# jhuldr/BrainFM

Measured on AMD Instinct MI355X. Metric: voxels/sec whole-volume multi-task inference, 256^3 tiled, higher is better.
Workload: dtype f16x3-split (fp32-grade); 1 GPU; 256^3 volume, reference tiling win160/stride80 -> 27 tiles, UNet3D f64 x6 levels, 9 heads (69 ch), fused tail + deformed atlas + on-device stitch of 17 keys; stitched_keys=17, mfma_passes=3, submission=hipGraph replay per tile shape, parallelism=tiles sharded over 1 rank(s), gather to rank 0, tiles_in_flight_per_gpu=2

## Files before the change

### brainfm_amd/csrc/conv3d_wino.hip

```cpp
#include "wino_shared.h"
#include <cstdlib>
#include <type_traits>

namespace {

typedef _Float16 half8 __attribute__((ext_vector_type(8)));
typedef _Float16 half4 __attribute__((ext_vector_type(4)));
typedef float floatx16 __attribute__((ext_vector_type(16)));

constexpr int KC = 16;
constexpr int NTHR = 256;
constexpr int MLD = 33;

struct WinoParams {
    const float* A;
    int CA, D, H, W;
    const float *scale, *shift, *bound;
    int G;
    const uint4* wp;
    int wexp, Cout;
    float slope;
    float* out;
    int accum;
    int TD, TH, TW, HT, PW;
// ... 530 lines not shown
        *reinterpret_cast<float4*>(p.pool_out + dbase + off1) = v1;
    }
    if (tid < 64) {
        const size_t d = (size_t)mt * p.Cout + nt * 64 + tid, s = (size_t)rp * p.Cout + nt * 64 + tid;
        if (p.rsum != nullptr) { p.rsum[d] = p.rsum[s]; p.rsq[d] = p.rsq[s]; p.rmn[d] = p.rmn[s]; p.rmx[d] = p.rmx[s]; }
        if (p.prsum != nullptr) { p.prsum[d] = p.prsum[s]; p.prsq[d] = p.prsq[s]; p.prmn[d] = p.prmn[s]; p.prmx[d] = p.prmx[s]; }
    }
}

template <class Pred>
__device__ __forceinline__ int wino_compact(int nMt, Pred pred, int* __restrict__ list, int* sh) {
    const int tid = threadIdx.x, lane = tid & 63, wv = tid >> 6;
    if (tid == 0) sh[16] = 0;
    __syncthreads();
    for (int b0 = 0; b0 < nMt; b0 += 1024) {
        const int mt = b0 + tid;
        const bool keep = mt < nMt && pred(mt);
        const unsigned long long bal = __ballot(keep);
        const int before = __popcll(bal & ((1ull << lane) - 1ull));
        if (lane == 0) sh[wv] = __popcll(bal);
        __syncthreads();
        int off = sh[16];
        for (int w = 0; w < wv; ++w) off += sh[w];
        if (keep) list[off + before] = mt;
        __syncthreads();
        if (tid == 0) {
            int t = 0;
            for (int w = 0; w < 16; ++w) t += sh[w];
            sh[16] += t;
        }
        __syncthreads();
    }
    return sh[16];
}

__global__ void __launch_bounds__(256) wino_box_active_kernel(const float* __restrict__ img, int D, int H, int W, int TD,
                                                               int TH, int TW, int nTy, int nTx, int nMt,
                                                               unsigned char* __restrict__ act) {
    const int mt = blockIdx.x * 4 + (threadIdx.x >> 6), lane = threadIdx.x & 63;
    if (mt >= nMt) return;
    const int tx = mt % nTx, ty = (mt / nTx) % nTy, tz = mt / (nTx * nTy);
    const int z0 = tz * TD, y0 = ty * TH, x0 = tx * TW;
    const int thw = TH * TW;
    bool nz = false;
    for (int q = lane; q < TD * thw; q += 64) {
        const int d = q / thw, r = q - d * thw, h = r / TW, w = r - h * TW;
        const int gz = z0 + d, gy = y0 + h, gx = x0 + w;
        if (gz < D && gy < H && gx < W) nz = nz || img[((int64_t)gz * H + gy) * W + gx] != 0.f;
    }
    const bool any = __any(nz);
    if (lane == 0) act[mt] = any ? 1 : 0;
}

__global__ void __launch_bounds__(1024) wino_mask_list_kernel(const unsigned char* __restrict__ act, int nMt,
                                                               int* __restrict__ list, int* __restrict__ n_out) {
    __shared__ int sh[17];
    const int n = wino_compact(nMt, [&](int mt) { return act[mt] != 0; }, list, sh);
    if (threadIdx.x == 0) n_out[0] = n;
}

__global__ void __launch_bounds__(256) uniform_boxes_kernel(const float* __restrict__ img, int D, int H, int W, int TD, int TH,
                                                            int TW, int nTz, int nTy, int nTx, int L, int R,
                                                            unsigned char* __restrict__ flags) {
    const int mt = blockIdx.x;
    const int tx = mt % nTx, ty = (mt / nTx) % nTy, tz = mt / (nTx * nTy);
    const int z0 = max(((tz * TD) << L) - R, 0), y0 = max(((ty * TH) << L) - R, 0), x0 = max(((tx * TW) << L) - R, 0);
    const int z1 = min((((tz + 1) * TD) << L) + R, D), y1 = min((((ty + 1) * TH) << L) + R, H);
    const int x1 = min((((tx + 1) * TW) << L) + R, W);
    const int ed = z1 - z0, eh = y1 - y0, ew = x1 - x0;
    int bad = 0;
    const unsigned ref = __float_as_uint(img[((int64_t)z0 * H + y0) * W + x0]);
    for (int q = threadIdx.x; q < ed * eh * ew; q += 256) {
        const int w = q % ew, r = q / ew, h = r % eh, d = r / eh;
        bad |= __float_as_uint(img[((int64_t)(z0 + d) * H + (y0 + h)) * W + (x0 + w)]) != ref ? 1 : 0;
    }
    bad = __syncthreads_or(bad);
    if (threadIdx.x == 0) {
        const int cz = tz == 0 ? 0 : (tz == nTz - 1 ? 2 : 1), cy = ty == 0 ? 0 : (ty == nTy - 1 ? 2 : 1);
        const int cx = tx == 0 ? 0 : (tx == nTx - 1 ? 2 : 1);
        const int dl = (D >> L) << L, hl = (H >> L) << L, wl = (W >> L) << L;
        const bool far = (tz != nTz - 1 && ((((tz + 1) * TD) << L) + R > dl)) ||
                         (ty != nTy - 1 && ((((ty + 1) * TH) << L) + R > hl)) ||
                         (tx != nTx - 1 && ((((tx + 1) * TW) << L) + R > wl));
        flags[mt] = bad || far ? 0 : (unsigned char)(1 + 9 * cz + 3 * cy + cx);
    }
}

constexpr int UL_COMP_WORDS = 4096;
template <bool AGENT>
__device__ __forceinline__ void uniform_lists_body(const unsigned char* flags, int n, int nTz, int nTy, int nTx,
                                                   int* __restrict__ first, int* __restrict__ cnt, int* __restrict__ rest,
                                                   int* __restrict__ uni, int* __restrict__ ncnt, int* __restrict__ nlist,
                                                   unsigned char* __restrict__ need, int* sh, int* fst, unsigned* comp) {
    auto flag = [&](int i) -> int {
        if constexpr (AGENT) return __hip_atomic_load(flags + i, __ATOMIC_RELAXED, __HIP_MEMORY_SCOPE_AGENT);
        else return flags[i];
    };
    const bool table = n <= UL_COMP_WORDS * 32;
    if (threadIdx.x < 27) fst[threadIdx.x] = n;
    if (table)
        for (int i = threadIdx.x; i < (n + 31) / 32; i += 1024) comp[i] = 0u;
    __syncthreads();
    for (int i = threadIdx.x; i < n; i += 1024) {
        const int f = flag(i);
        if (f != 0) atomicMin(&fst[f - 1], i);
    }
    __syncthreads();
    if (threadIdx.x < 27) first[threadIdx.x] = fst[threadIdx.x];
    const int n0 = wino_compact(n, [&](int mt) {
        const int f = flag(mt);
        const bool c = f == 0 || fst[f - 1] == mt;
        if (c && table) atomicOr(&comp[mt >> 5], 1u << (mt & 31));
        return c;
    }, rest, sh);
    if (threadIdx.x == 0) cnt[0] = n0;
    __syncthreads();
    auto computed = [&](int i) -> bool {
        if (table) return ((comp[i >> 5] >> (i & 31)) & 1u) != 0u;
        const int f = flag(i);
        return f == 0 || fst[f - 1] == i;
    };
    const int n1 = wino_compact(n, [&](int mt) { return !computed(mt); }, uni, sh);
    if (threadIdx.x == 0) cnt[1] = n1;
    __syncthreads();
    const int n2 = wino_compact(n, [&](int mt) {
        bool nd = false;
        if (!computed(mt)) {
            const int tx = mt % nTx, ty = (mt / nTx) % nTy, tz = mt / (nTx * nTy);
            for (int dz = -1; dz <= 1; ++dz)
                for (int dy = -1; dy <= 1; ++dy)
                    for (int dx = -1; dx <= 1; ++dx) {
                        const int z = tz + dz, y = ty + dy, x = tx + dx;
                        if (z >= 0 && z < nTz && y >= 0 && y < nTy && x >= 0 && x < nTx)
                            nd = nd || computed((z * nTy + y) * nTx + x);
                    }
        }
        need[mt] = nd ? 1 : 0;
        return nd;
    }, nlist, sh);
    if (threadIdx.x == 0) ncnt[0] = n2;
}

__global__ void __launch_bounds__(1024) uniform_lists_kernel(const unsigned char* __restrict__ flags, int n, int nTz, int nTy,
                                                             int nTx, int* __restrict__ first, int* __restrict__ cnt,
                                                             int* __restrict__ rest, int* __restrict__ uni,
                                                             int* __restrict__ ncnt, int* __restrict__ nlist,
                                                             unsigned char* __restrict__ need) {
    __shared__ int sh[17];
    __shared__ int fst[27];
    __shared__ unsigned comp[UL_COMP_WORDS];
    uniform_lists_body<false>(flags, n, nTz, nTy, nTx, first, cnt, rest, uni, ncnt, nlist, need, sh, fst, comp);
}

constexpr int UL_MAX = 4;
constexpr int UL_LOADS = 8;
struct UniLevel {
    int TD, TH, TW, nTz, nTy, nTx, L, R;
    int n, per, wg0;
    unsigned char* flags;
    int* first;
};
struct UniLevels {
    const float* img;
    int D, H, W, nlev, nwg;
    int* ticket;
    UniLevel lv[UL_MAX];
};

__global__ void __launch_bounds__(1024) uniform_levels_kernel(const UniLevels p) {
    __shared__ int sh[17];
    __shared__ int fst[27];
    __shared__ int bad_w[16];
    __shared__ int is_last;
    __shared__ unsigned comp[UL_COMP_WORDS];
    const int tid = threadIdx.x, grp = tid >> 8, t = tid & 255;
    int li = 0;
    for (int i = 1; i < p.nlev; ++i)
        if ((int)blockIdx.x >= p.lv[i].wg0) li = i;
    const UniLevel& v = p.lv[li];
    const int D = p.D, H = p.H, W = p.W, L = v.L, R = v.R;
    const int box0 = ((int)blockIdx.x - v.wg0) * 4 * v.per;
    for (int r = 0; r < v.per; ++r) {
        const int mt = box0 + r * 4 + grp;
        const bool live = mt < v.n;
        int bad = 0;
        int tx = 0, ty = 0, tz = 0;
        if (live) {
            tx = mt % v.nTx; ty = (mt / v.nTx) % v.nTy; tz = mt / (v.nTx * v.nTy);
            const int z0 = max(((tz * v.TD) << L) - R, 0), y0 = max(((ty * v.TH) << L) - R, 0);
            const int x0 = max(((tx * v.TW) << L) - R, 0);
            const int z1 = min((((tz + 1) * v.TD) << L) + R, D), y1 = min((((ty + 1) * v.TH) << L) + R, H);
            const int x1 = min((((tx + 1) * v.TW) << L) + R, W);
            const int eh = y1 - y0, ew = x1 - x0, nq = (z1 - z0) * eh * ew;
            const unsigned ref = __float_as_uint(p.img[((int64_t)z0 * H + y0) * W + x0]);
            int w = t % ew, h = (t / ew) % eh, d = (t / ew) / eh;
            const int sw = 256 % ew, sh_ = (256 / ew) % eh, sd = (256 / ew) / eh;
            const float* const base = p.img + ((int64_t)z0 * H + y0) * W + x0;
            for (int qb = 0; qb < nq && !bad; qb += UL_LOADS * 256) {
                unsigned val[UL_LOADS];
#pragma unroll
                for (int k = 0; k < UL_LOADS; ++k) {
                    val[k] = ref;
                    if (qb + k * 256 + t < nq) val[k] = __float_as_uint(base[(unsigned)(d * H + h) * (unsigned)W + (unsigned)w]);
                    w += sw;
                    if (w >= ew) { w -= ew; ++h; }
                    h += sh_;
                    if (h >= eh) { h -= eh; ++d; }
                    d += sd;
                }
                int diff = 0;
#pragma unroll
                for (int k = 0; k < UL_LOADS; ++k) diff |= val[k] != ref ? 1 : 0;
                bad = __any(diff) ? 1 : 0;
            }
        }
        if ((tid & 63) == 0) bad_w[tid >> 6] = bad;
        __syncthreads();
        if (live && t == 0) {
            const int any_bad = bad_w[grp * 4] | bad_w[grp * 4 + 1] | bad_w[grp * 4 + 2] | bad_w[grp * 4 + 3];
            const int cz = tz == 0 ? 0 : (tz == v.nTz - 1 ? 2 : 1), cy = ty == 0 ? 0 : (ty == v.nTy - 1 ? 2 : 1);
            const int cx = tx == 0 ? 0 : (tx == v.nTx - 1 ? 2 : 1);
            const int dl = (D >> L) << L, hl = (H >> L) << L, wl = (W >> L) << L;
            const bool far = (tz != v.nTz - 1 && ((((tz + 1) * v.TD) << L) + R > dl)) ||
                             (ty != v.nTy - 1 && ((((ty + 1) * v.TH) << L) + R > hl)) ||
                             (tx != v.nTx - 1 && ((((tx + 1) * v.TW) << L) + R > wl));
            __hip_atomic_store(v.flags + mt, any_bad || far ? (unsigned char)0 : (unsigned char)(1 + 9 * cz + 3 * cy + cx),
                               __ATOMIC_RELAXED, __HIP_MEMORY_SCOPE_AGENT);
        }
        __syncthreads();
    }
    asm volatile("s_waitcnt vmcnt(0)" ::: "memory");
    __syncthreads();
    if (tid == 0) {
        const int got = __hip_atomic_fetch_add(p.ticket, 1, __ATOMIC_RELEASE, __HIP_MEMORY_SCOPE_AGENT);
        is_last = got == p.nwg - 1;
        if (is_last) __hip_atomic_store(p.ticket, 0, __ATOMIC_RELAXED, __HIP_MEMORY_SCOPE_AGENT);
    }
    __syncthreads();
    if (!is_last) return;
    __builtin_amdgcn_fence(__ATOMIC_ACQUIRE, "agent");
    for (int i = 0; i < p.nlev; ++i) {
        const int n = p.lv[i].n;
        const UniformFlagBuf fb{p.lv[i].flags, (size_t)n};
        uniform_lists_body<true>(fb.flags, n, p.lv[i].nTz, p.lv[i].nTy, p.lv[i].nTx, fb.first(), fb.counts(), fb.rest_list(),
                                 fb.uniform_list(), fb.need_count(), fb.need_list(), fb.need(), sh, fst, comp);
        __syncthreads();
    }
}

__global__ void pack_wino(const float* __restrict__ w, int Cin, int Cout, int wexp, int npl, uint4* __restrict__ out) {
    const int KCN = Cin / KC;
    const int nf = 2 * npl;
    const int64_t n = (int64_t)(Cout / 64) * 4 * KCN * 9 * nf * 64;
    const float s = ldexpf(1.0f, wexp);
    for (int64_t i = (int64_t)blockIdx.x * blockDim.x + threadIdx.x; i < n; i += (int64_t)gridDim.x * blockDim.x) {
        const int lane = (int)(i & 63);
        int64_t r = i >> 6;
        const int f = (int)(r % nf); r /= nf;
        const int t = (int)(r % 9); r /= 9;
        const int kc = (int)(r % KCN); r /= KCN;
        const int ps = (int)(r & 3); r >>= 2;
        const int ntile = (int)r;
        const int nb = f / npl, hl = f - nb * npl;
        const int co = ntile * 64 + nb * 32 + (lane & 31);
        const int ci0 = kc * KC + 8 * (lane >> 5);
        half8 v;
#pragma unroll
        for (int j = 0; j < 8; ++j) {
            const float* g = w + ((size_t)co * Cin + ci0 + j) * 27 + t * 3;
            const float g0 = g[0], g1 = g[1], g2 = g[2];
            const float u = ps == 0 ? g0 : ps == 1 ? ((g0 + g1) + g2) * 0.5f : ps == 2 ? ((g0 - g1) + g2) * 0.5f : g2;
            const float x = u * s;
            const _Float16 hh = (_Float16)x;
            v[j] = hl == 0 ? hh : (_Float16)(x - (float)hh);
        }
        out[i] = __builtin_bit_cast(uint4, v);
    }
}

constexpr int PKW_ROW = KC * 27 + 1;
__global__ void __launch_bounds__(256) pack_wino_tiled(const float* __restrict__ w, int Cin, int Cout, int wexp, int npl,
                                                       uint4* __restrict__ out) {
    extern __shared__ float pkw_lds[];
    const int KCN = Cin / KC;
    const int nf = 2 * npl;
    const int nb = blockIdx.x & 1;
    const int kc = (blockIdx.x >> 1) % KCN, ntile = (blockIdx.x >> 1) / KCN;
    const float s = ldexpf(1.0f, wexp);
    const float* src0 = w + ((int64_t)(ntile * 64 + nb * 32) * Cin + kc * KC) * 27;
    bfm_stage_rows<32, KC * 27, PKW_ROW, 256>(src0, (int64_t)Cin * 27, pkw_lds, 1.0f,
                                              ((reinterpret_cast<uintptr_t>(w) & 15) == 0) && (Cin & 3) == 0);
    __syncthreads();
    const int lane = threadIdx.x & 63, wave = threadIdx.x >> 6;
    for (int q = wave; q < 4 * 9; q += 4) {
        const int t = q % 9;
        const int ps = q / 9;
        const float* src = pkw_lds + (lane & 31) * PKW_ROW + (8 * (lane >> 5)) * 27 + t * 3;
        half8 vh, vl;
// ... 336 lines not shown
```

### brainfm_amd/csrc/gn_stats.hip

```cpp
#include "bfm_common.h"

namespace {

constexpr int TPB = 256;

struct RepView {
    int d, h, w;
    const int32_t *rd, *rh, *rw;
};

__device__ __forceinline__ double vox_weight(const RepView& r, int64_t v) {
    if (r.rd == nullptr) return 1.0;
    int x = (int)(v % r.w);
    int64_t t = v / r.w;
    int y = (int)(t % r.h);
    int z = (int)(t / r.h);
    return (double)r.rd[z] * (double)r.rh[y] * (double)r.rw[x];
}

template <int VEC>
struct Acc {
    double s[VEC], q[VEC];
    float mn[VEC], mx[VEC];
    __device__ void init() {
// ... 63 lines not shown
    const int RP = TPB / CV;
    const bool active = t < RP * CV;
    const int r0 = t / CV, col = t % CV;
    Acc<VEC> a; a.init();
    if (active) {
        int64_t v = v0 + r0;
        for (; v + 3 * (int64_t)RP < v1; v += 4 * (int64_t)RP) {
            float x0[VEC], x1[VEC], x2[VEC], x3[VEC];
            load_vec<VEC>(X + v * C + (size_t)col * VEC, x0);
            load_vec<VEC>(X + (v + RP) * C + (size_t)col * VEC, x1);
            load_vec<VEC>(X + (v + 2 * (int64_t)RP) * C + (size_t)col * VEC, x2);
            load_vec<VEC>(X + (v + 3 * (int64_t)RP) * C + (size_t)col * VEC, x3);
            a.add(x0, vox_weight(rep, v));
            a.add(x1, vox_weight(rep, v + RP));
            a.add(x2, vox_weight(rep, v + 2 * (int64_t)RP));
            a.add(x3, vox_weight(rep, v + 3 * (int64_t)RP));
        }
        for (; v < v1; v += RP) {
            float x[VEC];
            load_vec<VEC>(X + v * C + (size_t)col * VEC, x);
            a.add(x, vox_weight(rep, v));
        }
    }
    double* ls = smem_d;
    double* lq = ls + (size_t)RP * C;
    float* lmn = reinterpret_cast<float*>(lq + (size_t)RP * C);
    float* lmx = lmn + (size_t)RP * C;
    if (active) {
#pragma unroll
        for (int i = 0; i < VEC; ++i) {
            int idx = r0 * C + col * VEC + i;
            ls[idx] = a.s[i]; lq[idx] = a.q[i]; lmn[idx] = a.mn[i]; lmx[idx] = a.mx[i];
        }
    }
    __syncthreads();
    for (int c = t; c < C; c += TPB) {
        double s = 0.0, q = 0.0; float mn = INFINITY, mx = -INFINITY;
        for (int r = 0; r < RP; ++r) {
            s += ls[r * C + c]; q += lq[r * C + c];
            mn = fminf(mn, lmn[r * C + c]); mx = fmaxf(mx, lmx[r * C + c]);
        }
        psum[row + c] = s; psq[row + c] = q; pmin[row + c] = mn; pmax[row + c] = mx;
    }
}

struct PartTab {
    const double *psum, *psq;
    const float *pmin, *pmax;
    int nb, C;
    double wgt;
};

constexpr int RR_MAX = 128;

__global__ void __launch_bounds__(TPB) rows_reduce(const double* __restrict__ rsum, const double* __restrict__ rsq,
                                                   const float* __restrict__ rmn, const float* __restrict__ rmx,
                                                   int nrows, int C, int rows_per_block, double* __restrict__ psum,
                                                   double* __restrict__ psq, float* __restrict__ pmin,
                                                   float* __restrict__ pmax) {
    extern __shared__ double smem_d[];
    const int t = threadIdx.x;
    const int r0 = blockIdx.x * rows_per_block;
    const int r1 = min(nrows, r0 + rows_per_block);
    const int CP = C < TPB ? C : TPB;
    const int RP = TPB / CP;
    double* ls = smem_d;
    double* lq = ls + TPB;
    float* lmn = reinterpret_cast<float*>(lq + TPB);
    float* lmx = lmn + TPB;
    for (int cb = 0; cb < C; cb += CP) {
        const int col = cb + t % CP, part = t / CP;
        double sv = 0.0, qv = 0.0;
        float mn = INFINITY, mx = -INFINITY;
        if (part < RP && col < C) {
            for (int r = r0 + part; r < r1; r += RP) {
                const size_t i = (size_t)r * C + col;
                sv += rsum[i]; qv += rsq[i];
                mn = fminf(mn, rmn[i]); mx = fmaxf(mx, rmx[i]);
            }
        }
        ls[t] = sv; lq[t] = qv; lmn[t] = mn; lmx[t] = mx;
        __syncthreads();
        if (part == 0 && col < C) {
            for (int pp = 1; pp < RP; ++pp) {
                const int i = pp * CP + (t % CP);
                sv += ls[i]; qv += lq[i];
                mn = fminf(mn, lmn[i]); mx = fmaxf(mx, lmx[i]);
            }
            const size_t o = (size_t)blockIdx.x * C + col;
            psum[o] = sv; psq[o] = qv; pmin[o] = mn; pmax[o] = mx;
        }
        __syncthreads();
    }
}

__device__ __forceinline__ void group_affine(int g, int cpg, int c_first, double count_per_channel, float eps,
                                             const float* __restrict__ gamma, const float* __restrict__ beta,
                                             float* __restrict__ scale, float* __restrict__ shift,
                                             float* __restrict__ bound, float* __restrict__ mean_out,
                                             float* __restrict__ rstd_out, const double* chan_s, const double* chan_q,
                                             const float* chan_mn, const float* chan_mx, float* red_mx) {
    const int t = threadIdx.x;
    __shared__ float sh_mean, sh_rstd;
    if (t < 64) {
        double S = 0.0, Q = 0.0;
        for (int c = t; c < cpg; c += 64) { S += chan_s[c]; Q += chan_q[c]; }
        S = wave_reduce_sum(S);
        Q = wave_reduce_sum(Q);
        if (t == 0) {
            double n = count_per_channel * (double)cpg;
            double mean = S / n;
            double var = Q / n - mean * mean;
            if (var < 0.0) var = 0.0;
            sh_mean = (float)mean;
            sh_rstd = (float)(1.0 / sqrt(var + (double)eps));
            if (mean_out) mean_out[g] = sh_mean;
            if (rstd_out) rstd_out[g] = sh_rstd;
        }
    }
    __syncthreads();
    const float mean = sh_mean, rstd = sh_rstd;
    float bmax = 0.f;
    for (int cg = t; cg < cpg; cg += TPB) {
        int c = c_first + cg;
        float sc = rstd * gamma[c];
        float sh = -sc * mean + beta[c];
        scale[c] = sc; shift[c] = sh;
        float b0 = fabsf(fmaf(chan_mn[cg], sc, sh));
        float b1 = fabsf(fmaf(chan_mx[cg], sc, sh));
        bmax = fmaxf(bmax, fmaxf(b0, b1));
    }
    bmax = wave_reduce_max(bmax);
// ... 7 lines not shown
}

constexpr int KS = 16;

template <typename T>
__device__ __forceinline__ T ld_agent(const T* p) { return __hip_atomic_load(p, __ATOMIC_RELAXED, __HIP_MEMORY_SCOPE_AGENT); }
template <typename T>
__device__ __forceinline__ void st_agent(T* p, T v) { __hip_atomic_store(p, v, __ATOMIC_RELAXED, __HIP_MEMORY_SCOPE_AGENT); }

struct RowsSrc {
    const double *rsum, *rsq;
    const float *rmn, *rmx;
    int nrows, C;
    double wgt;
};

__global__ void __launch_bounds__(TPB) rows_group_finalize(RowsSrc sa, RowsSrc sb, int G, double count_per_channel, float eps,
                                                           const float* __restrict__ gamma, const float* __restrict__ beta,
                                                           float* __restrict__ scale, float* __restrict__ shift,
                                                           float* __restrict__ bound, float* __restrict__ mean_out,
                                                           float* __restrict__ rstd_out, double* __restrict__ psum,
                                                           double* __restrict__ psq, float* __restrict__ pmn,
                                                           float* __restrict__ pmx, int* __restrict__ tickets) {
    extern __shared__ double smem_d[];
    __shared__ int is_last;
    const int t = threadIdx.x;
    const int g = blockIdx.x, k = blockIdx.y;
    const int Ctot = sa.C + sb.C;
    const int cpg = Ctot / G;
    const int c_first = g * cpg;
    double* chan_s = smem_d;
    double* chan_q = chan_s + cpg;
    double* red_s = chan_q + cpg;
    double* red_q = red_s + TPB;
    float* chan_mn = reinterpret_cast<float*>(red_q + TPB);
    float* chan_mx = chan_mn + cpg;
    float* red_mn = chan_mx + cpg;
    float* red_mx = red_mn + TPB;

    const int CP = cpg < TPB ? cpg : TPB;
    const int RP = TPB / CP;
    const bool active = t < RP * CP;
    const int cl = t % CP, part = t / CP;
    for (int cb = 0; cb < cpg; cb += CP) {
        const int cg = cb + cl;
        double sv = 0.0, qv = 0.0;
        float mn = INFINITY, mx = -INFINITY;
        if (active && cg < cpg) {
            const int c = c_first + cg;
            const RowsSrc& S = (c < sa.C) ? sa : sb;
            const int cc = (c < sa.C) ? c : c - sa.C;
            const int per = (S.nrows + KS - 1) / KS;
            const int r0 = k * per, r1 = min(S.nrows, r0 + per);
            for (int r = r0 + part; r < r1; r += RP) {
                const size_t i = (size_t)r * S.C + cc;
                sv += S.rsum[i]; qv += S.rsq[i];
                mn = fminf(mn, S.rmn[i]); mx = fmaxf(mx, S.rmx[i]);
            }
        }
        red_s[t] = sv; red_q[t] = qv; red_mn[t] = mn; red_mx[t] = mx;
        __syncthreads();
        if (active && part == 0 && cg < cpg) {
            for (int pp = 1; pp < RP; ++pp) {
                const int i = pp * CP + cl;
                sv += red_s[i]; qv += red_q[i];
                mn = fminf(mn, red_mn[i]); mx = fmaxf(mx, red_mx[i]);
            }
            const size_t o = ((size_t)g * KS + k) * cpg + cg;
            st_agent(psum + o, sv); st_agent(psq + o, qv); st_agent(pmn + o, mn); st_agent(pmx + o, mx);
        }
        __syncthreads();
    }
    asm volatile("s_waitcnt vmcnt(0)" ::: "memory");
    __syncthreads();
    if (t == 0) {
        const int got = __hip_atomic_fetch_add(tickets + g, 1, __ATOMIC_RELEASE, __HIP_MEMORY_SCOPE_AGENT);
        is_last = got == KS - 1;
        if (is_last) __hip_atomic_store(tickets + g, 0, __ATOMIC_RELAXED, __HIP_MEMORY_SCOPE_AGENT);
    }
    __syncthreads();
    if (!is_last) return;
    __builtin_amdgcn_fence(__ATOMIC_ACQUIRE, "agent");
    for (int cg = t; cg < cpg; cg += TPB) {
        const int c = c_first + cg;
        const double w = (c < sa.C) ? sa.wgt : sb.wgt;
        double ps[KS], pq[KS];
        float pn[KS], px[KS];
#pragma unroll
        for (int kk = 0; kk < KS; ++kk) {
            const size_t o = ((size_t)g * KS + kk) * cpg + cg;
            ps[kk] = ld_agent(psum + o); pq[kk] = ld_agent(psq + o); pn[kk] = ld_agent(pmn + o); px[kk] = ld_agent(pmx + o);
        }
        double sv = 0.0, qv = 0.0;
        float mn = INFINITY, mx = -INFINITY;
#pragma unroll
        for (int kk = 0; kk < KS; ++kk) { sv += ps[kk]; qv += pq[kk]; mn = fminf(mn, pn[kk]); mx = fmaxf(mx, px[kk]); }
        chan_s[cg] = sv * w; chan_q[cg] = qv * w; chan_mn[cg] = mn; chan_mx[cg] = mx;
    }
    __syncthreads();
    group_affine(g, cpg, c_first, count_per_channel, eps, gamma, beta, scale, shift, bound, mean_out, rstd_out, chan_s, chan_q,
                 chan_mn, chan_mx, red_mx);
}

__global__ void __launch_bounds__(TPB) gn_finalize(PartTab ta, PartTab tb, int G, double count_per_channel,
                                                   float eps, const float* __restrict__ gamma,
                                                   const float* __restrict__ beta, float* __restrict__ scale,
                                                   float* __restrict__ shift, float* __restrict__ bound,
                                                   float* __restrict__ mean_out, float* __restrict__ rstd_out) {
    extern __shared__ double smem_d[];
    const int t = threadIdx.x;
    const int g = blockIdx.x;
    const int Ctot = ta.C + tb.C;
    const int cpg = Ctot / G;
    const int c_first = g * cpg;
    if (blockIdx.y) {
        const size_t oa = (size_t)blockIdx.y * ta.nb * ta.C, ob = (size_t)blockIdx.y * tb.nb * tb.C;
        ta.psum += oa; ta.psq += oa; ta.pmin += oa; ta.pmax += oa;
        if (tb.C) { tb.psum += ob; tb.psq += ob; tb.pmin += ob; tb.pmax += ob; }
        scale += (size_t)blockIdx.y * Ctot; shift += (size_t)blockIdx.y * Ctot; bound += (size_t)blockIdx.y * G;
        if (mean_out) mean_out += (size_t)blockIdx.y * G;
        if (rstd_out) rstd_out += (size_t)blockIdx.y * G;
    }

    double* chan_s = smem_d;
    double* chan_q = chan_s + cpg;
    double* red_s = chan_q + cpg;
    double* red_q = red_s + TPB;
    float* chan_mn = reinterpret_cast<float*>(red_q + TPB);
    float* chan_mx = chan_mn + cpg;
    float* red_mn = chan_mx + cpg;
    float* red_mx = red_mn + TPB;

    const int cpgP = cpg < TPB ? cpg : TPB;
    const int P = TPB / cpgP;
    const bool active = t < P * cpgP;
    const int cl = t % cpgP, part = t / cpgP;

    for (int cb = 0; cb < cpg; cb += cpgP) {
        const int cg = cb + cl;
        double s = 0.0, q = 0.0; float mn = INFINITY, mx = -INFINITY;
        if (active && cg < cpg) {
            int c = c_first + cg;
            const PartTab& T = (c < ta.C) ? ta : tb;
            int cc = (c < ta.C) ? c : c - ta.C;
            for (int b = part; b < T.nb; b += P) {
                size_t i = (size_t)b * T.C + cc;
                s += T.psum[i]; q += T.psq[i];
                mn = fminf(mn, T.pmin[i]); mx = fmaxf(mx, T.pmax[i]);
            }
            s *= T.wgt; q *= T.wgt;
        }
        red_s[t] = s; red_q[t] = q; red_mn[t] = mn; red_mx[t] = mx;
        __syncthreads();
        if (active && part == 0 && cg < cpg) {
            for (int p = 1; p < P; ++p) {
                int i = p * cpgP + cl;
                s += red_s[i]; q += red_q[i];
                mn = fminf(mn, red_mn[i]); mx = fmaxf(mx, red_mx[i]);
            }
            chan_s[cg] = s; chan_q[cg] = q; chan_mn[cg] = mn; chan_mx[cg] = mx;
        }
        __syncthreads();
    }

    group_affine(g, cpg, c_first, count_per_channel, eps, gamma, beta, scale, shift, bound, mean_out, rstd_out, chan_s, chan_q,
                 chan_mn, chan_mx, red_mx);
}

struct Plan {
    int nbA, nbB;
    int64_t vpbA, vpbB;
    size_t offA_sum, offA_sq, offA_mn, offA_mx, offB_sum, offB_sq, offB_mn, offB_mx, total;
};

int blocks_for(int64_t nvox, int C, int64_t* vpb) {
    int64_t nb = 32768 / C;
    if (nb > 2048) nb = 2048;
    if (nb < 8) nb = 8;
    int64_t by_vox = bfm_cdiv64(nvox, 16);
    if (nb > by_vox) nb = by_vox;
    if (nb < 1) nb = 1;
    *vpb = bfm_cdiv64(nvox, nb);
    nb = bfm_cdiv64(nvox, *vpb);
    return (int)nb;
}

Plan make_plan(int CA, int CB, int64_t nvoxA, int64_t nvoxB, int S = 1) {
    Plan p{};
    p.nbA = blocks_for(nvoxA, CA, &p.vpbA);
    size_t off = 0;
    auto take = [&](size_t bytes) { size_t o = off; off += (bytes + 255) & ~(size_t)255; return o; };
    p.offA_sum = take((size_t)S * p.nbA * CA * 8); p.offA_sq = take((size_t)S * p.nbA * CA * 8);
    p.offA_mn = take((size_t)S * p.nbA * CA * 4); p.offA_mx = take((size_t)S * p.nbA * CA * 4);
    if (CB > 0) {
        p.nbB = blocks_for(nvoxB, CB, &p.vpbB);
        p.offB_sum = take((size_t)S * p.nbB * CB * 8); p.offB_sq = take((size_t)S * p.nbB * CB * 8);
        p.offB_mn = take((size_t)S * p.nbB * CB * 4); p.offB_mx = take((size_t)S * p.nbB * CB * 4);
    }
    p.total = off;
    return p;
}

// ... 287 lines not shown
```

Measured before the change: 222.5 million voxels/s.

## Blocked bitmask list compaction and unrolled GroupNorm row folding

Replaces the per-element lambda compaction in the mask-list and uniform-list kernels with a blocked scheme. Each thread owns a contiguous run of flags, reads them in packed words, and builds bitmask tables in shared memory, so a single block scan replaces repeated compaction rounds and the neighbour test becomes bit operations on rows. The GroupNorm reductions gain an 8-way unrolled row fold that issues independent loads together to hide latency. In exchange the code adds shared memory (a second 4096-word table), an occupancy hint on the levels kernel, and more complex edge handling, which raises the risk of subtle ordering bugs.

```diff
diff --git a/brainfm_amd/csrc/conv3d_wino.hip b/brainfm_amd/csrc/conv3d_wino.hip
--- a/brainfm_amd/csrc/conv3d_wino.hip
+++ b/brainfm_amd/csrc/conv3d_wino.hip
@@ -606,10 +606,96 @@
     if (lane == 0) act[mt] = any ? 1 : 0;
 }
 
+constexpr int UL_GROUP = 16;
+
+struct OwnBoxes {
+    int per, b0, b1;
+    bool wide;
+    __device__ OwnBoxes(const unsigned char* flags, int n) {
+        per = (n + 1023) >> 10;
+        b0 = min(n, (int)threadIdx.x * per);
+        b1 = min(n, b0 + per);
+        wide = (per & 3) == 0 && (reinterpret_cast<uintptr_t>(flags) & 3) == 0;
+    }
+};
+
+template <bool AGENT>
+__device__ __forceinline__ void flag_group(const unsigned char* flags, int g0, int b1, bool wide, unsigned (&w)[UL_GROUP / 4]) {
+    if (wide) {
+#pragma unroll
+        for (int k = 0; k < UL_GROUP / 4; ++k) {
+            w[k] = 0u;
+            if (g0 + 4 * k < b1) {
+                const unsigned* q = reinterpret_cast<const unsigned*>(flags + g0 + 4 * k);
+                if constexpr (AGENT) w[k] = __hip_atomic_load(q, __ATOMIC_RELAXED, __HIP_MEMORY_SCOPE_AGENT);
+                else w[k] = *q;
+                const int rem = b1 - (g0 + 4 * k);
+                if (rem < 4) w[k] &= (1u << (8 * rem)) - 1u;
+            }
+        }
+    } else {
+        unsigned b[UL_GROUP];
+#pragma unroll
+        for (int k = 0; k < UL_GROUP; ++k) {
+            b[k] = 0u;
+            if (g0 + k < b1) {
+                if constexpr (AGENT) b[k] = __hip_atomic_load(flags + g0 + k, __ATOMIC_RELAXED, __HIP_MEMORY_SCOPE_AGENT);
+                else b[k] = flags[g0 + k];
+            }
+        }
+#pragma unroll
+        for (int k = 0; k < UL_GROUP / 4; ++k) w[k] = b[4 * k] | (b[4 * k + 1] << 8) | (b[4 * k + 2] << 16) | (b[4 * k + 3] << 24);
+    }
+}
+__device__ __forceinline__ int flag_of(const unsigned (&w)[UL_GROUP / 4], int k) { return (int)((w[k >> 2] >> (8 * (k & 3))) & 255u); }
+
+__device__ __forceinline__ int block_scan_1024(int v, int* sh, int& total) {
+    const int lane = threadIdx.x & 63, wv = threadIdx.x >> 6;
+    int inc = v;
+#pragma unroll
+    for (int d = 1; d < 64; d <<= 1) {
+        const int o = __shfl_up(inc, d);
+        if (lane >= d) inc += o;
+    }
+    __syncthreads();
+    if (lane == 63) sh[wv] = inc;
+    __syncthreads();
+    int off = 0, tot = 0;
+#pragma unroll
+    for (int w = 0; w < 16; ++w) {
+        const int s = sh[w];
+        off += w < wv ? s : 0;
+        tot += s;
+    }
+    total = tot;
+    return off + inc - v;
+}
+
+__device__ __forceinline__ int wino_compact_blocked(const unsigned char* __restrict__ flags, int n, int* __restrict__ list,
+                                                    int* sh) {
+    const OwnBoxes o(flags, n);
+    unsigned w[UL_GROUP / 4] = {0u, 0u, 0u, 0u};
+    int cnt = 0;
+    for (int g0 = o.b0; g0 < o.b1; g0 += UL_GROUP) {
+        flag_group<false>(flags, g0, o.b1, o.wide, w);
+#pragma unroll
+        for (int k = 0; k < UL_GROUP; ++k) cnt += flag_of(w, k) != 0 ? 1 : 0;
+    }
+    int total;
+    int off = block_scan_1024(cnt, sh, total);
+    for (int g0 = o.b0; g0 < o.b1; g0 += UL_GROUP) {
+        if (o.per > UL_GROUP) flag_group<false>(flags, g0, o.b1, o.wide, w);
+#pragma unroll
+        for (int k = 0; k < UL_GROUP; ++k)
+            if (flag_of(w, k) != 0) list[off++] = g0 + k;
+    }
+    return total;
+}
+
 __global__ void __launch_bounds__(1024) wino_mask_list_kernel(const unsigned char* __restrict__ act, int nMt,
                                                                int* __restrict__ list, int* __restrict__ n_out) {
-    __shared__ int sh[17];
-    const int n = wino_compact(nMt, [&](int mt) { return act[mt] != 0; }, list, sh);
+    __shared__ int sh[16];
+    const int n = wino_compact_blocked(act, nMt, list, sh);
     if (threadIdx.x == 0) n_out[0] = n;
 }
 
@@ -642,10 +728,10 @@
 
 constexpr int UL_COMP_WORDS = 4096;
 template <bool AGENT>
-__device__ __forceinline__ void uniform_lists_body(const unsigned char* flags, int n, int nTz, int nTy, int nTx,
-                                                   int* __restrict__ first, int* __restrict__ cnt, int* __restrict__ rest,
-                                                   int* __restrict__ uni, int* __restrict__ ncnt, int* __restrict__ nlist,
-                                                   unsigned char* __restrict__ need, int* sh, int* fst, unsigned* comp) {
+__device__ __forceinline__ void uniform_lists_rounds(const unsigned char* flags, int n, int nTz, int nTy, int nTx,
+                                                     int* __restrict__ first, int* __restrict__ cnt, int* __restrict__ rest,
+                                                     int* __restrict__ uni, int* __restrict__ ncnt, int* __restrict__ nlist,
+                                                     unsigned char* __restrict__ need, int* sh, int* fst, unsigned* comp) {
     auto flag = [&](int i) -> int {
         if constexpr (AGENT) return __hip_atomic_load(flags + i, __ATOMIC_RELAXED, __HIP_MEMORY_SCOPE_AGENT);
         else return flags[i];
@@ -695,6 +781,114 @@
     if (threadIdx.x == 0) ncnt[0] = n2;
 }
 
+__device__ __forceinline__ unsigned table_bits(const unsigned* tab, int a, int cnt) {
+    const int s = a & 31;
+    unsigned v = tab[a >> 5] >> s;
+    if (s + cnt > 32) v |= tab[(a >> 5) + 1] << (32 - s);
+    return cnt >= 32 ? v : v & ((1u << cnt) - 1u);
+}
+__device__ __forceinline__ void table_or(unsigned* tab, int a, unsigned m) {
+    const int s = a & 31;
+    if ((m << s) != 0u) atomicOr(&tab[a >> 5], m << s);
+    if (s > 16 && (m >> (32 - s)) != 0u) atomicOr(&tab[(a >> 5) + 1], m >> (32 - s));
+}
+
+template <bool AGENT>
+__device__ __forceinline__ void uniform_lists_body(const unsigned char* flags, int n, int nTz, int nTy, int nTx,
+                                                   int* __restrict__ first, int* __restrict__ cnt, int* __restrict__ rest,
+                                                   int* __restrict__ uni, int* __restrict__ ncnt, int* __restrict__ nlist,
+                                                   unsigned char* __restrict__ need, int* sh, int* fst, unsigned* comp,
+                                                   unsigned* ndb, unsigned (&w)[UL_GROUP / 4], bool have_w) {
+    if (n > UL_COMP_WORDS * 32) {
+        uniform_lists_rounds<AGENT>(flags, n, nTz, nTy, nTx, first, cnt, rest, uni, ncnt, nlist, need, sh, fst, comp);
+        return;
+    }
+    const int tid = threadIdx.x;
+    const OwnBoxes o(flags, n);
+    if (tid < 27) fst[tid] = n;
+    for (int i = tid; i < (n + 31) / 32; i += 1024) { comp[i] = 0u; ndb[i] = 0u; }
+    __syncthreads();
+    unsigned seen = 0u;
+    for (int g0 = o.b0; g0 < o.b1; g0 += UL_GROUP) {
+        if (!(have_w && g0 == o.b0)) flag_group<AGENT>(flags, g0, o.b1, o.wide, w);
+#pragma unroll
+        for (int k = 0; k < UL_GROUP; ++k) {
+            const int f = flag_of(w, k);
+            if (f != 0 && ((seen >> (f - 1)) & 1u) == 0u) {
+                seen |= 1u << (f - 1);
+                atomicMin(&fst[f - 1], g0 + k);
+            }
+        }
+    }
+    __syncthreads();
+    if (tid < 27) first[tid] = fst[tid];
+    int c0 = 0;
+    for (int g0 = o.b0; g0 < o.b1; g0 += UL_GROUP) {
+        if (o.per > UL_GROUP) flag_group<AGENT>(flags, g0, o.b1, o.wide, w);
+        unsigned m = 0u;
+#pragma unroll
+        for (int k = 0; k < UL_GROUP; ++k) {
+            const int f = flag_of(w, k);
+            if (g0 + k < o.b1 && (f == 0 || fst[f - 1] == g0 + k)) m |= 1u << k;
+        }
+        c0 += __popc(m);
+        table_or(comp, g0, m);
+    }
+    int n0;
+    int off0 = block_scan_1024(c0, sh, n0);
+    int off1 = o.b0 - off0;
+    if (tid == 0) { cnt[0] = n0; cnt[1] = n - n0; }
+    int tx = o.b0 % nTx, ty = (o.b0 / nTx) % nTy, tz = o.b0 / (nTx * nTy);
+    int c2 = 0;
+    for (int g0 = o.b0; g0 < o.b1; g0 += UL_GROUP) {
+        const int ng = min(UL_GROUP, o.b1 - g0);
+        const unsigned cb = table_bits(comp, g0, ng);
+        for (int k = 0; k < ng; ++k) {
+            if ((cb >> k) & 1u) rest[off0++] = g0 + k;
+            else uni[off1++] = g0 + k;
+        }
+        unsigned nm = 0u;
+        for (int k = 0; k < ng;) {
+            const int len = min(ng - k, nTx - tx);
+            const int lo = max(tx - 1, 0), nx = min(tx + len, nTx - 1) - lo + 1;
+            unsigned near = 0u;
+            for (int z = max(tz - 1, 0); z <= min(tz + 1, nTz - 1); ++z)
+                for (int y = max(ty - 1, 0); y <= min(ty + 1, nTy - 1); ++y) {
+                    const unsigned b = table_bits(comp, (z * nTy + y) * nTx + lo, nx);
+                    near |= b | (b >> 1) | (b << 1);
+                }
+            nm |= ((near >> (tx - lo)) & ((1u << len) - 1u)) << k;
+            k += len;
+            tx += len;
+            if (tx == nTx) { tx = 0; if (++ty == nTy) { ty = 0; ++tz; } }
+        }
+        nm &= ~cb;
+        c2 += __popc(nm);
+        table_or(ndb, g0, nm);
+#pragma unroll
+        for (int q = 0; q < UL_GROUP / 4; ++q) {
+            const unsigned b = (nm >> (4 * q)) & 15u;
+            if (o.wide && 4 * q + 3 < ng) {
+                *reinterpret_cast<unsigned*>(need + g0 + 4 * q) = (b & 1u) | ((b & 2u) << 7) | ((b & 4u) << 14) | ((b & 8u) << 21);
+            } else {
+#pragma unroll
+                for (int k = 4 * q; k < 4 * q + 4; ++k)
+                    if (k < ng) need[g0 + k] = (unsigned char)((nm >> k) & 1u);
+            }
+        }
+    }
+    int n2;
+    int off2 = block_scan_1024(c2, sh, n2);
+    if (tid == 0) ncnt[0] = n2;
+    for (int g0 = o.b0; g0 < o.b1; g0 += UL_GROUP) {
+        unsigned nm = table_bits(ndb, g0, min(UL_GROUP, o.b1 - g0));
+        while (nm != 0u) {
+            nlist[off2++] = g0 + __ffs(nm) - 1;
+            nm &= nm - 1u;
+        }
+    }
+}
+
 __global__ void __launch_bounds__(1024) uniform_lists_kernel(const unsigned char* __restrict__ flags, int n, int nTz, int nTy,
                                                              int nTx, int* __restrict__ first, int* __restrict__ cnt,
                                                              int* __restrict__ rest, int* __restrict__ uni,
@@ -703,10 +897,14 @@
     __shared__ int sh[17];
     __shared__ int fst[27];
     __shared__ unsigned comp[UL_COMP_WORDS];
-    uniform_lists_body<false>(flags, n, nTz, nTy, nTx, first, cnt, rest, uni, ncnt, nlist, need, sh, fst, comp);
+    __shared__ unsigned ndb[UL_COMP_WORDS];
+    unsigned w[UL_GROUP / 4] = {0u, 0u, 0u, 0u};
+    uniform_lists_body<false>(flags, n, nTz, nTy, nTx, first, cnt, rest, uni, ncnt, nlist, need, sh, fst, comp, ndb, w, false);
 }
 
 constexpr int UL_MAX = 4;
+constexpr int UL_PRE = 2;
+static_assert(UL_PRE == 2 && UL_PRE <= UL_MAX, "uniform_levels_kernel selects a level's preloaded flags between two");
 constexpr int UL_LOADS = 8;
 struct UniLevel {
     int TD, TH, TW, nTz, nTy, nTx, L, R;
@@ -721,12 +919,13 @@
     UniLevel lv[UL_MAX];
 };
 
-__global__ void __launch_bounds__(1024) uniform_levels_kernel(const UniLevels p) {
+__global__ void __launch_bounds__(1024, 8) uniform_levels_kernel(const UniLevels p) {
     __shared__ int sh[17];
     __shared__ int fst[27];
     __shared__ int bad_w[16];
     __shared__ int is_last;
     __shared__ unsigned comp[UL_COMP_WORDS];
+    __shared__ unsigned ndb[UL_COMP_WORDS];
     const int tid = threadIdx.x, grp = tid >> 8, t = tid & 255;
     int li = 0;
     for (int i = 1; i < p.nlev; ++i)
@@ -793,11 +992,24 @@
     __syncthreads();
     if (!is_last) return;
     __builtin_amdgcn_fence(__ATOMIC_ACQUIRE, "agent");
+    unsigned wl[UL_PRE][UL_GROUP / 4];
+#pragma unroll
+    for (int i = 0; i < UL_PRE; ++i) {
+#pragma unroll
+        for (int k = 0; k < UL_GROUP / 4; ++k) wl[i][k] = 0u;
+        if (i < p.nlev) {
+            const OwnBoxes o(p.lv[i].flags, p.lv[i].n);
+            flag_group<true>(p.lv[i].flags, o.b0, o.b1, o.wide, wl[i]);
+        }
+    }
     for (int i = 0; i < p.nlev; ++i) {
         const int n = p.lv[i].n;
         const UniformFlagBuf fb{p.lv[i].flags, (size_t)n};
+        unsigned w[UL_GROUP / 4];
+#pragma unroll
+        for (int k = 0; k < UL_GROUP / 4; ++k) w[k] = i == 0 ? wl[0][k] : wl[1][k];
         uniform_lists_body<true>(fb.flags, n, p.lv[i].nTz, p.lv[i].nTy, p.lv[i].nTx, fb.first(), fb.counts(), fb.rest_list(),
-                                 fb.uniform_list(), fb.need_count(), fb.need_list(), fb.need(), sh, fst, comp);
+                                 fb.uniform_list(), fb.need_count(), fb.need_list(), fb.need(), sh, fst, comp, ndb, w, i < UL_PRE);
         __syncthreads();
     }
 }
diff --git a/brainfm_amd/csrc/gn_stats.hip b/brainfm_amd/csrc/gn_stats.hip
--- a/brainfm_amd/csrc/gn_stats.hip
+++ b/brainfm_amd/csrc/gn_stats.hip
@@ -139,6 +139,36 @@
 };
 
 constexpr int RR_MAX = 128;
+
+constexpr int FOLD_U = 8;
+
+__device__ __forceinline__ void fold_rows(const double* __restrict__ rsum, const double* __restrict__ rsq,
+                                          const float* __restrict__ rmn, const float* __restrict__ rmx, int C, int col, int r,
+                                          int r1, int step, double& sv, double& qv, float& mn, float& mx) {
+    double s[FOLD_U], q[FOLD_U];
+    float n[FOLD_U], x[FOLD_U];
+    for (; r1 - r > (FOLD_U - 1) * step; r += FOLD_U * step) {
+#pragma unroll
+        for (int u = 0; u < FOLD_U; ++u) {
+            const size_t i = (size_t)(r + u * step) * C + col;
+            s[u] = rsum[i]; q[u] = rsq[i]; n[u] = rmn[i]; x[u] = rmx[i];
+        }
+#pragma unroll
+        for (int u = 0; u < FOLD_U; ++u) { sv += s[u]; qv += q[u]; mn = fminf(mn, n[u]); mx = fmaxf(mx, x[u]); }
+    }
+    if (r < r1) {
+#pragma unroll
+        for (int u = 0; u < FOLD_U - 1; ++u) {
+            if (r + u * step < r1) {
+                const size_t i = (size_t)(r + u * step) * C + col;
+                s[u] = rsum[i]; q[u] = rsq[i]; n[u] = rmn[i]; x[u] = rmx[i];
+            }
+        }
+#pragma unroll
+        for (int u = 0; u < FOLD_U - 1; ++u)
+            if (r + u * step < r1) { sv += s[u]; qv += q[u]; mn = fminf(mn, n[u]); mx = fmaxf(mx, x[u]); }
+    }
+}
 
 __global__ void __launch_bounds__(TPB) rows_reduce(const double* __restrict__ rsum, const double* __restrict__ rsq,
                                                    const float* __restrict__ rmn, const float* __restrict__ rmx,
@@ -160,11 +190,7 @@
         double sv = 0.0, qv = 0.0;
         float mn = INFINITY, mx = -INFINITY;
         if (part < RP && col < C) {
-            for (int r = r0 + part; r < r1; r += RP) {
-                const size_t i = (size_t)r * C + col;
-                sv += rsum[i]; qv += rsq[i];
-                mn = fminf(mn, rmn[i]); mx = fmaxf(mx, rmx[i]);
-            }
+            fold_rows(rsum, rsq, rmn, rmx, C, col, r0 + part, r1, RP, sv, qv, mn, mx);
         }
         ls[t] = sv; lq[t] = qv; lmn[t] = mn; lmx[t] = mx;
         __syncthreads();
@@ -278,11 +304,7 @@
             const int cc = (c < sa.C) ? c : c - sa.C;
             const int per = (S.nrows + KS - 1) / KS;
             const int r0 = k * per, r1 = min(S.nrows, r0 + per);
-            for (int r = r0 + part; r < r1; r += RP) {
-                const size_t i = (size_t)r * S.C + cc;
-                sv += S.rsum[i]; qv += S.rsq[i];
-                mn = fminf(mn, S.rmn[i]); mx = fmaxf(mx, S.rmx[i]);
-            }
+            fold_rows(S.rsum, S.rsq, S.rmn, S.rmx, S.C, cc, r0 + part, r1, RP, sv, qv, mn, mx);
         }
         red_s[t] = sv; red_q[t] = qv; red_mn[t] = mn; red_mx[t] = mx;
         __syncthreads();
@@ -369,11 +391,7 @@
             int c = c_first + cg;
             const PartTab& T = (c < ta.C) ? ta : tb;
             int cc = (c < ta.C) ? c : c - ta.C;
-            for (int b = part; b < T.nb; b += P) {
-                size_t i = (size_t)b * T.C + cc;
-                s += T.psum[i]; q += T.psq[i];
-                mn = fminf(mn, T.pmin[i]); mx = fmaxf(mx, T.pmax[i]);
-            }
+            fold_rows(T.psum, T.psq, T.pmin, T.pmax, T.C, cc, part, T.nb, P, s, q, mn, mx);
             s *= T.wgt; q *= T.wgt;
         }
         red_s[t] = s; red_q[t] = q; red_mn[t] = mn; red_mx[t] = mx;
```

New measurement: 224.3 million voxels/s, median of 6. About the same (+0.8%).

## Build uniform-tile lists in LDS with per-thread chunks and bitmask neighbour tests

Applied to the files above, without the earlier changes.

Adds an LDS-resident path for building the uniform/rest/need tile lists when the tile count fits a cap. Flags are loaded once into shared memory, each thread owns a contiguous chunk, and first-occurrence, computed-bitmask, neighbour-dilation and compaction are done with bit operations and one packed wave prefix scan. This replaces several global-memory compaction rounds with atomics. It also pins the levels kernel's waves per EU and makes the last-block test wave-uniform. It raises LDS use per block and adds an untimed debug macro that skips list building.

```diff
diff --git a/brainfm_amd/csrc/conv3d_wino.hip b/brainfm_amd/csrc/conv3d_wino.hip
--- a/brainfm_amd/csrc/conv3d_wino.hip
+++ b/brainfm_amd/csrc/conv3d_wino.hip
@@ -642,10 +642,10 @@
 
 constexpr int UL_COMP_WORDS = 4096;
 template <bool AGENT>
-__device__ __forceinline__ void uniform_lists_body(const unsigned char* flags, int n, int nTz, int nTy, int nTx,
-                                                   int* __restrict__ first, int* __restrict__ cnt, int* __restrict__ rest,
-                                                   int* __restrict__ uni, int* __restrict__ ncnt, int* __restrict__ nlist,
-                                                   unsigned char* __restrict__ need, int* sh, int* fst, unsigned* comp) {
+__device__ __forceinline__ void uniform_lists_rounds(const unsigned char* flags, int n, int nTz, int nTy, int nTx,
+                                                     int* __restrict__ first, int* __restrict__ cnt, int* __restrict__ rest,
+                                                     int* __restrict__ uni, int* __restrict__ ncnt, int* __restrict__ nlist,
+                                                     unsigned char* __restrict__ need, int* sh, int* fst, unsigned* comp) {
     auto flag = [&](int i) -> int {
         if constexpr (AGENT) return __hip_atomic_load(flags + i, __ATOMIC_RELAXED, __HIP_MEMORY_SCOPE_AGENT);
         else return flags[i];
@@ -695,15 +695,166 @@
     if (threadIdx.x == 0) ncnt[0] = n2;
 }
 
+constexpr int UL_CAP = 16384;
+struct UniListsLds {
+    int sh[17];
+    int fst[27];
+    union {
+        unsigned comp[UL_COMP_WORDS];
+        struct {
+            unsigned bits[UL_CAP / 32 + 2];
+            unsigned short stage[UL_CAP];
+        } l;
+    };
+    unsigned lf[UL_CAP / 4];
+    unsigned long long wsum[16];
+};
+static_assert(UL_CAP % 4096 == 0 && UL_CAP / 1024 + 2 <= 32 && UL_CAP <= 65536, "a chunk's row window fits one word, a box 16 bits");
+
+template <bool AGENT>
+__device__ __forceinline__ void uniform_lists_lds(const unsigned char* flags, int n, int nTz, int nTy, int nTx,
+                                                  int* __restrict__ first, int* __restrict__ cnt, int* __restrict__ rest,
+                                                  int* __restrict__ uni, int* __restrict__ ncnt, int* __restrict__ nlist,
+                                                  unsigned char* __restrict__ need, UniListsLds& s) {
+    const int tid = threadIdx.x, lane = tid & 63, wv = tid >> 6;
+    unsigned char* const lfb = reinterpret_cast<unsigned char*>(s.lf);
+    const int nw = (n + 3) >> 2;
+    {
+        unsigned v[UL_CAP / 4096];
+#pragma unroll
+        for (int k = 0; k < UL_CAP / 4096; ++k) {
+            const int w = k * 1024 + tid;
+            v[k] = 0u;
+            if (w < nw) {
+                const unsigned* const src = reinterpret_cast<const unsigned*>(flags) + w;
+                if constexpr (AGENT) v[k] = __hip_atomic_load(src, __ATOMIC_RELAXED, __HIP_MEMORY_SCOPE_AGENT);
+                else v[k] = *src;
+            }
+        }
+#pragma unroll
+        for (int k = 0; k < UL_CAP / 4096; ++k)
+            if (k * 1024 + tid < nw) s.lf[k * 1024 + tid] = v[k];
+    }
+    if (tid < 27) s.fst[tid] = n;
+    for (int w = tid; w < (n >> 5) + 2; w += 1024) s.l.bits[w] = 0u;
+    __syncthreads();
+    const int c = (n + 1023) >> 10, i0 = min(tid * c, n), i1 = min(i0 + c, n);
+    unsigned seen = 0u;
+#pragma clang loop vectorize(disable) unroll(disable)
+    for (int i = i0; i < i1; ++i) {
+        const int f = lfb[i];
+        if (f != 0 && !((seen >> f) & 1u)) {
+            seen |= 1u << f;
+            atomicMin(&s.fst[f - 1], i);
+        }
+    }
+    __syncthreads();
+    if (tid < 27) first[tid] = s.fst[tid];
+    unsigned cm = 0u;
+#pragma clang loop vectorize(disable) unroll(disable)
+    for (int i = i0; i < i1; ++i) {
+        const int f = lfb[i];
+        if (f == 0 || s.fst[f - 1] == i) cm |= 1u << (i - i0);
+    }
+    if (cm != 0u) {
+        const unsigned long long wide = (unsigned long long)cm << (i0 & 31);
+        const unsigned lo = (unsigned)wide, hi = (unsigned)(wide >> 32);
+        if (lo != 0u) atomicOr(&s.l.bits[i0 >> 5], lo);
+        if (hi != 0u) atomicOr(&s.l.bits[(i0 >> 5) + 1], hi);
+    }
+    __syncthreads();
+    unsigned nm = 0u;
+    {
+        int tx = i0 % nTx, ty = (i0 / nTx) % nTy, tz = i0 / (nTx * nTy);
+        for (int i = i0; i < i1;) {
+            const int seg = min(i1 - i, nTx - tx);
+            const unsigned mates = ~(cm >> (i - i0)) & ((1u << seg) - 1u);
+            if (mates != 0u) {
+                const int x0 = max(tx - 1, 0), len = min(tx + seg, nTx - 1) - x0 + 1;
+                unsigned acc = 0u;
+#pragma unroll 1
+                for (int dz = -1; dz <= 1; ++dz)
+                    for (int dy = -1; dy <= 1; ++dy) {
+                        const int z = tz + dz, y = ty + dy;
+                        if (z >= 0 && z < nTz && y >= 0 && y < nTy) {
+                            const int b = (z * nTy + y) * nTx + x0;
+                            acc |= (unsigned)((((unsigned long long)s.l.bits[(b >> 5) + 1] << 32) | s.l.bits[b >> 5]) >> (b & 31));
+                        }
+                    }
+                acc &= (1u << len) - 1u;
+                const unsigned near = acc | (acc << 1) | (acc >> 1);
+                nm |= ((near >> (tx - x0)) & mates) << (i - i0);
+            }
+            i += seg;
+            tx += seg;
+            if (tx == nTx) {
+                tx = 0;
+                if (++ty == nTy) { ty = 0; ++tz; }
+            }
+        }
+#pragma clang loop vectorize(disable) unroll(disable)
+        for (int i = i0; i < i1; ++i) lfb[i] = (nm >> (i - i0)) & 1u;
+    }
+    const unsigned long long r = __popc(cm), d = __popc(nm), m = (unsigned long long)(i1 - i0) - r;
+    const unsigned long long v = r | (m << 21) | (d << 42);
+    unsigned long long inc = v;
+    for (int o = 1; o < 64; o <<= 1) {
+        const unsigned long long up = __shfl_up(inc, o);
+        if (lane >= o) inc += up;
+    }
+    if (lane == 63) s.wsum[wv] = inc;
+    __syncthreads();
+    unsigned long long base = 0ull, tot = 0ull;
+    for (int w = 0; w < 16; ++w) {
+        const unsigned long long t = s.wsum[w];
+        if (w < wv) base += t;
+        tot += t;
+    }
+    const unsigned long long ex = base + inc - v;
+    int ro = (int)(ex & 0x1fffffull), mo = (int)((ex >> 21) & 0x1fffffull), no = (int)(ex >> 42);
+    if (tid == 0) {
+        cnt[0] = (int)(tot & 0x1fffffull);
+        cnt[1] = (int)((tot >> 21) & 0x1fffffull);
+        ncnt[0] = (int)(tot >> 42);
+    }
+    const int n0 = (int)(tot & 0x1fffffull), n2 = (int)(tot >> 42);
+#pragma clang loop vectorize(disable) unroll(disable)
+    for (int i = i0; i < i1; ++i) {
+        if ((cm >> (i - i0)) & 1u) s.l.stage[ro++] = (unsigned short)i;
+        else s.l.stage[n0 + mo++] = (unsigned short)i;
+    }
+    __syncthreads();
+    for (int k = tid; k < n; k += 1024) {
+        const int b = s.l.stage[k];
+        if (k < n0) rest[k] = b;
+        else uni[k - n0] = b;
+    }
+    __syncthreads();
+#pragma clang loop vectorize(disable) unroll(disable)
+    for (int i = i0; i < i1; ++i)
+        if ((nm >> (i - i0)) & 1u) s.l.stage[no++] = (unsigned short)i;
+    __syncthreads();
+    for (int k = tid; k < n2; k += 1024) nlist[k] = s.l.stage[k];
+    for (int w = tid; w < (n >> 2); w += 1024) reinterpret_cast<unsigned*>(need)[w] = s.lf[w];
+    if (tid < (n & 3)) need[(n & ~3) + tid] = lfb[(n & ~3) + tid];
+}
+
+template <bool AGENT>
+__device__ __forceinline__ void uniform_lists_body(const unsigned char* flags, int n, int nTz, int nTy, int nTx,
+                                                   int* __restrict__ first, int* __restrict__ cnt, int* __restrict__ rest,
+                                                   int* __restrict__ uni, int* __restrict__ ncnt, int* __restrict__ nlist,
+                                                   unsigned char* __restrict__ need, UniListsLds& s) {
+    if (n <= UL_CAP) uniform_lists_lds<AGENT>(flags, n, nTz, nTy, nTx, first, cnt, rest, uni, ncnt, nlist, need, s);
+    else uniform_lists_rounds<AGENT>(flags, n, nTz, nTy, nTx, first, cnt, rest, uni, ncnt, nlist, need, s.sh, s.fst, s.comp);
+}
+
 __global__ void __launch_bounds__(1024) uniform_lists_kernel(const unsigned char* __restrict__ flags, int n, int nTz, int nTy,
                                                              int nTx, int* __restrict__ first, int* __restrict__ cnt,
                                                              int* __restrict__ rest, int* __restrict__ uni,
                                                              int* __restrict__ ncnt, int* __restrict__ nlist,
                                                              unsigned char* __restrict__ need) {
-    __shared__ int sh[17];
-    __shared__ int fst[27];
-    __shared__ unsigned comp[UL_COMP_WORDS];
-    uniform_lists_body<false>(flags, n, nTz, nTy, nTx, first, cnt, rest, uni, ncnt, nlist, need, sh, fst, comp);
+    __shared__ UniListsLds s;
+    uniform_lists_body<false>(flags, n, nTz, nTy, nTx, first, cnt, rest, uni, ncnt, nlist, need, s);
 }
 
 constexpr int UL_MAX = 4;
@@ -721,12 +872,10 @@
     UniLevel lv[UL_MAX];
 };
 
-__global__ void __launch_bounds__(1024) uniform_levels_kernel(const UniLevels p) {
-    __shared__ int sh[17];
-    __shared__ int fst[27];
+__global__ void __launch_bounds__(1024) __attribute__((amdgpu_waves_per_eu(8, 8))) uniform_levels_kernel(const UniLevels p) {
     __shared__ int bad_w[16];
     __shared__ int is_last;
-    __shared__ unsigned comp[UL_COMP_WORDS];
+    __shared__ UniListsLds s;
     const int tid = threadIdx.x, grp = tid >> 8, t = tid & 255;
     int li = 0;
     for (int i = 1; i < p.nlev; ++i)
@@ -791,13 +940,16 @@
         if (is_last) __hip_atomic_store(p.ticket, 0, __ATOMIC_RELAXED, __HIP_MEMORY_SCOPE_AGENT);
     }
     __syncthreads();
-    if (!is_last) return;
+    if (!__builtin_amdgcn_readfirstlane(is_last)) return;
     __builtin_amdgcn_fence(__ATOMIC_ACQUIRE, "agent");
+#ifdef BFM_UL_NO_LISTS
+    return;
+#endif
     for (int i = 0; i < p.nlev; ++i) {
         const int n = p.lv[i].n;
         const UniformFlagBuf fb{p.lv[i].flags, (size_t)n};
         uniform_lists_body<true>(fb.flags, n, p.lv[i].nTz, p.lv[i].nTy, p.lv[i].nTx, fb.first(), fb.counts(), fb.rest_list(),
-                                 fb.uniform_list(), fb.need_count(), fb.need_list(), fb.need(), sh, fst, comp);
+                                 fb.uniform_list(), fb.need_count(), fb.need_list(), fb.need(), s);
         __syncthreads();
     }
 }
```

After: 223.3 million voxels/s before, 224.4 million voxels/s after (median of 6 runs). Within noise of the previous version (+0.5%).
